# bubustack/bobrapet

Measured on AMD Instinct MI355X. Metric: StoryRuns/sec + p50 step latency, 8-way parallel Story, higher is better.
Workload: dtype bf16; 1 GPU; bench_config=parallel8, global_batch=2165, seq_len=128, parallelism=single, engine=bobraccel-native, branches=8

## Files before the change

### bobrapet_amd/csrc/hip/bindings.cpp

```cpp
#include <torch/extension.h>

#include <c10/hip/HIPStream.h>
#include <hip/hip_runtime.h>

const void* bobra_native_lane_ptr();
bool bobra_native_tensor_get(const std::string& key, at::Tensor* out);
size_t bobra_native_registry_size();
void bobra_native_lane_stats(long*, long*, long*, std::string*);

extern "C" {
void launch_rmsnorm(void*, void*, void*, const void*, int, int, float, bool,
                    hipStream_t);
void launch_silu_mul(void*, const void*, const void*, long, hipStream_t);
void launch_rope(void*, void*, const void*, const void*, int, int, int, int,
                 hipStream_t);
void launch_embed_pool(void*, void*, const void*, const void*, int, int, int,
                       int, hipStream_t);
void launch_add_bf16(void*, const void*, const void*, long, hipStream_t);
void launch_attn_prefill(void*, const void*, const void*, const void*, int,
                         int, int, int, long, float, int, void*, hipStream_t);
void launch_silu_mul_strided(void*, const void*, const void*, long, int, long,
                             hipStream_t);
void launch_rope_qkv(void*, void*, const void*, const void*, const void*, int,
                     int, int, int, long, hipStream_t);
void launch_rope_qkv_decode(void*, void*, void*, const void*, const void*,
                            const void*, int, int, int, int, int, hipStream_t);
void launch_argmax_rows(void*, const void*, int, int, hipStream_t);
void launch_attn_decode(void*, void*, const void*, const void*, const void*,
                        int, int, int, int, int, const void*, float,
                        hipStream_t);
void launch_dbg_mfma(void*, const void*, const void*, hipStream_t);
void launch_attn_prefill_pipe(void*, const void*, const void*, const void*,
                              int, int, int, int, long, float, int, void*,
                              hipStream_t);
void launch_attn_prefill_qrope(void*, const void*, const void*, const void*,
                               int, int, int, int, long, long, const void*,
                               int, float, int, hipStream_t);
void launch_attn_prefill_variant(int, void*, const void*, const void*,
                                 const void*, int, int, int, int, float, int,
                                 hipStream_t);
void launch_gemm_bf16_nt(void*, const void*, const void*, int, int, int,
                         hipStream_t);
void launch_gemv_bf16_nt(void*, const void*, const void*, int, int, int,
                         hipStream_t);
void launch_gemm256(int, void*, const void*, const void*, const void*,
                    const void*, void*, int, int, int, float, float,
                    hipStream_t);
void launch_gemv2(int, void*, const void*, const void*, const void*, int, int,
                  int, float, float, hipStream_t);
void launch_gemm256b_disc(int, void*, const void*, const void*, int, int,
                          int, hipStream_t);
void launch_gemm256w(int, void*, const void*, const void*, const void*,
                     const void*, void*, int, int, int, float, float,
                     hipStream_t);
void launch_gemmsk(int, void*, void*, const void*, const void*, const void*,
                   const void*, void*, int, int, int, float, float,
                   hipStream_t);
long gemmsk_ws_elems(int, int);
void launch_gemm256b(int, void*, const void*, const void*, const void*,
                     const void*, void*, int, int, int, float, float,
                     hipStream_t);
void launch_rowsumsq(void*, const void*, int, int, hipStream_t);
void launch_dbg_attn_core(void*, void*, const void*, const void*, const void*,
                          hipStream_t);
}

namespace {

hipStream_t cur_stream() { return c10::hip::getCurrentHIPStream(); }

void check_bf16(const torch::Tensor& t, const char* name) {
  TORCH_CHECK(t.is_cuda(), name, " must be on the GPU");
  TORCH_CHECK(t.scalar_type() == torch::kBFloat16, name, " must be bf16");
  TORCH_CHECK(t.is_contiguous(), name, " must be contiguous");
}

torch::Tensor rmsnorm(torch::Tensor x, torch::Tensor w, double eps) {
  check_bf16(x, "x");
  check_bf16(w, "w");
  const int H = x.size(-1);
  TORCH_CHECK(H % 8 == 0 && H <= 8192, "rmsnorm: H must be %8==0 and <=8192");
  TORCH_CHECK(w.numel() == H, "rmsnorm: weight shape mismatch");
  auto out = torch::empty_like(x);
  const long rows = x.numel() / H;
  launch_rmsnorm(out.data_ptr(), x.data_ptr(), nullptr, w.data_ptr(),
                 (int)rows, H, (float)eps, false, cur_stream());
  return out;
}

torch::Tensor fused_add_rmsnorm(torch::Tensor x, torch::Tensor residual,
                                torch::Tensor w, double eps) {
  check_bf16(x, "x");
  check_bf16(residual, "residual");
  check_bf16(w, "w");
  const int H = x.size(-1);
  TORCH_CHECK(H % 8 == 0 && H <= 8192, "fused_add_rmsnorm: bad H");
  TORCH_CHECK(residual.sizes() == x.sizes(), "shape mismatch");
  auto out = torch::empty_like(x);
  const long rows = x.numel() / H;
  launch_rmsnorm(out.data_ptr(), x.data_ptr(), residual.data_ptr(),
                 w.data_ptr(), (int)rows, H, (float)eps, true, cur_stream());
  return out;
}

torch::Tensor silu_mul(torch::Tensor gate, torch::Tensor up) {
  check_bf16(gate, "gate");
  check_bf16(up, "up");
  TORCH_CHECK(gate.sizes() == up.sizes(), "silu_mul: shape mismatch");
  TORCH_CHECK(gate.numel() % 8 == 0, "silu_mul: numel must be %8==0");
  auto out = torch::empty_like(gate);
  launch_silu_mul(out.data_ptr(), gate.data_ptr(), up.data_ptr(), gate.numel(),
                  cur_stream());
  return out;
}

void rope_inplace(torch::Tensor q, torch::Tensor k, torch::Tensor cos_t,
                  torch::Tensor sin_t) {
  check_bf16(q, "q");
  check_bf16(k, "k");
  TORCH_CHECK(cos_t.scalar_type() == torch::kFloat32 && cos_t.is_contiguous(),
              "cos must be f32 contiguous");
  TORCH_CHECK(sin_t.scalar_type() == torch::kFloat32 && sin_t.is_contiguous(),
              "sin must be f32 contiguous");
  const int T = q.size(0), Hq = q.size(1), D = q.size(2);
  const int Hk = k.size(1);
  TORCH_CHECK(k.size(0) == T && k.size(2) == D, "rope: q/k shape mismatch");
  TORCH_CHECK(cos_t.size(0) == T && cos_t.size(1) == D / 2, "rope: table shape");
  launch_rope(q.data_ptr(), k.data_ptr(), cos_t.data_ptr(), sin_t.data_ptr(),
              T, Hq, Hk, D, cur_stream());
}

torch::Tensor embed_pool(torch::Tensor table, torch::Tensor ids) {
  check_bf16(table, "table");
  TORCH_CHECK(ids.scalar_type() == torch::kInt32 && ids.is_cuda() &&
                  ids.is_contiguous(),
              "ids must be int32 on GPU");
  const int V = table.size(0), H = table.size(1);
  const int B = ids.size(0), S = ids.size(1);
  TORCH_CHECK(H % 8 == 0 && H <= 8192, "embed_pool: bad H");
  auto out = torch::empty({B, H}, table.options());
  const int nchunk = (S + 7) / 8;
  auto pooled =
      torch::empty({(long)B * nchunk, H}, table.options().dtype(torch::kFloat32));
  if (H % 2048 != 0)
    (void)hipMemsetAsync(pooled.data_ptr(), 0,
                         (size_t)B * nchunk * H * sizeof(float), cur_stream());
  launch_embed_pool(out.data_ptr(), pooled.data_ptr(), table.data_ptr(),
                    ids.data_ptr(), B, S, H, V, cur_stream());
  return out;
}

torch::Tensor add_bf16(torch::Tensor a, torch::Tensor b) {
  check_bf16(a, "a");
  check_bf16(b, "b");
  TORCH_CHECK(a.sizes() == b.sizes() && a.numel() % 8 == 0, "add: bad shapes");
  auto out = torch::empty_like(a);
  launch_add_bf16(out.data_ptr(), a.data_ptr(), b.data_ptr(), a.numel(),
                  cur_stream());
  return out;
}

torch::Tensor attn_prefill(torch::Tensor q, torch::Tensor k, torch::Tensor v,
                           double scale, bool causal) {
  check_bf16(q, "q");
  check_bf16(k, "k");
  const int B = q.size(0), S = q.size(1), Hq = q.size(2), D = q.size(3);
  const int Hkv = k.size(2);
  TORCH_CHECK(D == 128, "attn_prefill: D must be 128");
  TORCH_CHECK(Hq % Hkv == 0, "attn_prefill: Hq must be a multiple of Hkv");
  TORCH_CHECK(k.size(1) == S && v.size(1) == S, "attn_prefill: S mismatch");
  TORCH_CHECK(v.is_cuda() && v.scalar_type() == torch::kBFloat16, "v dtype");
  TORCH_CHECK(v.stride(3) == 1 && v.stride(2) == D, "attn_prefill: v head must be contiguous");
  TORCH_CHECK(v.stride(0) == v.stride(1) * S, "attn_prefill: v batch stride");
  auto out = torch::empty_like(q);
  launch_attn_prefill(out.data_ptr(), q.data_ptr(), k.data_ptr(), v.data_ptr(),
                      B, Hq, Hkv, S, (long)v.stride(1), (float)scale,
                      causal ? 1 : 0, nullptr, cur_stream());
  return out;
}

torch::Tensor attn_prefill_qrope(torch::Tensor q, torch::Tensor k,
                                 torch::Tensor v, torch::Tensor inv_freq,
                                 int64_t pos0, double scale, bool causal) {
  check_bf16(k, "k");
  TORCH_CHECK(q.is_cuda() && q.scalar_type() == torch::kBFloat16, "q dtype");
  const int B = q.size(0), S = q.size(1), Hq = q.size(2), D = q.size(3);
  const int Hkv = k.size(2);
  TORCH_CHECK(D == 128, "attn_prefill_qrope: D must be 128");
  TORCH_CHECK(Hq % Hkv == 0, "attn_prefill_qrope: Hq % Hkv");
  TORCH_CHECK(k.size(1) == S && v.size(1) == S, "attn_prefill_qrope: S mismatch");
  TORCH_CHECK(q.stride(3) == 1 && q.stride(2) == D, "q head must be contiguous");
  TORCH_CHECK(q.stride(0) == q.stride(1) * S, "q batch stride");
  TORCH_CHECK(v.is_cuda() && v.scalar_type() == torch::kBFloat16, "v dtype");
  TORCH_CHECK(v.stride(3) == 1 && v.stride(2) == D, "v head must be contiguous");
  TORCH_CHECK(v.stride(0) == v.stride(1) * S, "v batch stride");
  TORCH_CHECK(inv_freq.is_cuda() && inv_freq.scalar_type() == torch::kFloat32 &&
                  inv_freq.numel() == D / 2 && inv_freq.is_contiguous(),
              "inv_freq must be f32 [D/2] contiguous");
  auto out = torch::empty({B, S, Hq, D}, k.options());
  launch_attn_prefill_qrope(out.data_ptr(), q.data_ptr(), k.data_ptr(),
                            v.data_ptr(), B, Hq, Hkv, S, (long)v.stride(1),
                            (long)q.stride(1), inv_freq.data_ptr(), (int)pos0,
                            (float)scale, causal ? 1 : 0, cur_stream());
  return out;
}

std::vector<torch::Tensor> rope_k_only(torch::Tensor qkv, int64_t Hq,
                                       int64_t Hk, int64_t D,
                                       torch::Tensor cos_t,
                                       torch::Tensor sin_t) {
  check_bf16(qkv, "qkv");
  const long T = qkv.size(0);
  TORCH_CHECK(qkv.is_contiguous(), "rope_k_only: qkv must be contiguous");
  TORCH_CHECK(cos_t.size(0) == T && cos_t.size(1) == D / 2, "rope_k_only tables");
  auto kout = torch::empty({T, Hk, D}, qkv.options());
  const unsigned short* base =
      (const unsigned short*)qkv.data_ptr() + (long)Hq * D;
  launch_rope_qkv(nullptr, kout.data_ptr(), base, cos_t.data_ptr(),
                  sin_t.data_ptr(), (int)T, 0, (int)Hk, (int)D,
                  (long)qkv.size(1), cur_stream());
  return {kout};
}

torch::Tensor attn_prefill_pipe(torch::Tensor q, torch::Tensor k,
                                torch::Tensor v, double scale, bool causal) {
  check_bf16(q, "q");
  check_bf16(k, "k");
  const int B = q.size(0), S = q.size(1), Hq = q.size(2), D = q.size(3);
  const int Hkv = k.size(2);
  TORCH_CHECK(D == 128, "attn_prefill_pipe: D must be 128");
  TORCH_CHECK(Hq % Hkv == 0, "attn_prefill_pipe: Hq % Hkv");
  TORCH_CHECK(k.size(1) == S && v.size(1) == S, "attn_prefill_pipe: S mismatch");
  TORCH_CHECK(v.is_cuda() && v.scalar_type() == torch::kBFloat16, "v dtype");
  TORCH_CHECK(v.stride(3) == 1 && v.stride(2) == D, "v head must be contiguous");
  TORCH_CHECK(v.stride(0) == v.stride(1) * S, "v batch stride");
  auto out = torch::empty_like(q);
  launch_attn_prefill_pipe(out.data_ptr(), q.data_ptr(), k.data_ptr(),
                           v.data_ptr(), B, Hq, Hkv, S, (long)v.stride(1),
                           (float)scale, causal ? 1 : 0, nullptr,
                           cur_stream());
  return out;
}

std::vector<torch::Tensor> attn_prefill_stats(torch::Tensor q, torch::Tensor k,
                                              torch::Tensor v, double scale,
                                              bool causal) {
  check_bf16(q, "q");
  check_bf16(k, "k");
  const int B = q.size(0), S = q.size(1), Hq = q.size(2), D = q.size(3);
  const int Hkv = k.size(2);
  TORCH_CHECK(D == 128, "attn_prefill_stats: D must be 128");
  TORCH_CHECK(Hq % Hkv == 0, "attn_prefill_stats: Hq % Hkv");
  TORCH_CHECK(v.stride(3) == 1 && v.stride(2) == D, "v head must be contiguous");
  auto out = torch::empty_like(q);
  auto stats = torch::empty({B, Hq, S, 2}, q.options().dtype(torch::kFloat32));
  launch_attn_prefill(out.data_ptr(), q.data_ptr(), k.data_ptr(), v.data_ptr(),
                      B, Hq, Hkv, S, (long)v.stride(1), (float)scale,
                      causal ? 1 : 0, stats.data_ptr(), cur_stream());
  return {out, stats};
}

torch::Tensor attn_decode(torch::Tensor q, torch::Tensor kc, torch::Tensor vc,
                          long L, double scale) {
  check_bf16(q, "q");
  check_bf16(kc, "kc");
  check_bf16(vc, "vc");
  const int B = q.size(0), Hq = q.size(1), D = q.size(2);
  const int Hkv = kc.size(1), Smax = kc.size(2);
  TORCH_CHECK(D == 128, "attn_decode: D must be 128");
  TORCH_CHECK(L <= Smax, "attn_decode: L > Smax");
  auto out = torch::empty_like(q);
  void* ws_ptr = nullptr;
  torch::Tensor ws;
  if (!(getenv("BOBRA_DEC_V1") && getenv("BOBRA_DEC_V1")[0] == '1') &&
      Hq / Hkv <= 8) {
    const int nchunk = (Smax + 255) / 256;
    ws = torch::empty({(long)B * Hkv * nchunk * 8 * 130},
                      q.options().dtype(torch::kFloat32));
    ws_ptr = ws.data_ptr();
  }
  launch_attn_decode(out.data_ptr(), ws_ptr, q.data_ptr(), kc.data_ptr(),
                     vc.data_ptr(), B, Hq, Hkv, Smax, (int)L, nullptr,
                     (float)scale, cur_stream());
  return out;
}

torch::Tensor attn_decode_t(torch::Tensor q, torch::Tensor kc,
                            torch::Tensor vc, torch::Tensor L_dev,
                            double scale) {
  check_bf16(q, "q");
  const int B = q.size(0), Hq = q.size(1), D = q.size(2);
  const int Hkv = kc.size(1), Smax = kc.size(2);
  TORCH_CHECK(D == 128, "attn_decode_t: D must be 128");
  TORCH_CHECK(L_dev.scalar_type() == torch::kInt32 && L_dev.is_cuda(),
              "L must be an int32 device scalar");
  auto out = torch::empty_like(q);
  void* ws_ptr = nullptr;
  torch::Tensor ws;
  if (!(getenv("BOBRA_DEC_V1") && getenv("BOBRA_DEC_V1")[0] == '1') &&
      Hq / Hkv <= 8) {
    const int nchunk = (Smax + 255) / 256;
    ws = torch::empty({(long)B * Hkv * nchunk * 8 * 130},
                      q.options().dtype(torch::kFloat32));
    ws_ptr = ws.data_ptr();
  }
  launch_attn_decode(out.data_ptr(), ws_ptr, q.data_ptr(), kc.data_ptr(),
                     vc.data_ptr(), B, Hq, Hkv, Smax, 0, L_dev.data_ptr(),
                     (float)scale, cur_stream());
  return out;
}

torch::Tensor rope_qkv_decode(torch::Tensor qkv, torch::Tensor kc,
                              torch::Tensor vc, torch::Tensor inv_freq,
                              torch::Tensor L_dev, long Hq, long Hkv, long D) {
  check_bf16(qkv, "qkv");
  check_bf16(kc, "kc");
  check_bf16(vc, "vc");
  const int B = qkv.size(0);
  const int Smax = kc.size(2);
  TORCH_CHECK(qkv.size(1) == (Hq + 2 * Hkv) * D, "rope_qkv_decode: row size");
  TORCH_CHECK(inv_freq.scalar_type() == torch::kFloat32 &&
                  inv_freq.is_contiguous() && inv_freq.numel() == D / 2,
              "inv_freq must be f32 [D/2] contiguous");
  TORCH_CHECK(L_dev.scalar_type() == torch::kInt32 && L_dev.is_cuda(),
              "L must be an int32 device scalar");
  auto q_out = torch::empty({(long)B, Hq, D}, qkv.options());
  launch_rope_qkv_decode(q_out.data_ptr(), kc.data_ptr(), vc.data_ptr(),
                         qkv.data_ptr(), inv_freq.data_ptr(), L_dev.data_ptr(),
                         B, (int)Hq, (int)Hkv, (int)D, Smax, cur_stream());
  return q_out;
}

torch::Tensor argmax_rows(torch::Tensor x) {
  check_bf16(x, "x");
  const int N = x.size(-1);
  const int M = x.numel() / N;
  auto ids = torch::empty({(long)M}, x.options().dtype(torch::kLong));
  launch_argmax_rows(ids.data_ptr(), x.data_ptr(), M, N, cur_stream());
  return ids;
}

torch::Tensor silu_mul_strided(torch::Tensor gate_up) {
  check_bf16(gate_up, "gate_up");
  const int two_i = gate_up.size(-1);
  const int inner = two_i / 2;
  TORCH_CHECK(inner % 8 == 0, "silu_mul_strided: I must be %8==0");
  const long rows = gate_up.numel() / two_i;
  auto sizes = gate_up.sizes().vec();
  sizes.back() = inner;
  auto out = torch::empty(sizes, gate_up.options());
  const unsigned short* base = (const unsigned short*)gate_up.data_ptr();
  launch_silu_mul_strided(out.data_ptr(), base, base + inner, rows, inner,
                          (long)two_i, cur_stream());
  return out;
}

std::vector<torch::Tensor> rope_qkv(torch::Tensor qkv, int Hq, int Hk, int D,
                                    torch::Tensor cos_t, torch::Tensor sin_t) {
  check_bf16(qkv, "qkv");
  const long T = qkv.size(0);
  TORCH_CHECK(cos_t.size(0) == T && cos_t.size(1) == D / 2, "rope_qkv tables");
  auto q = torch::empty({T, (long)Hq, (long)D}, qkv.options());
  auto k = torch::empty({T, (long)Hk, (long)D}, qkv.options());
  launch_rope_qkv(q.data_ptr(), k.data_ptr(), qkv.data_ptr(), cos_t.data_ptr(),
                  sin_t.data_ptr(), (int)T, Hq, Hk, D, (long)qkv.size(1),
                  cur_stream());
  return {q, k};
}

torch::Tensor gemm_nt(torch::Tensor a, torch::Tensor b) {
  check_bf16(a, "a");
  check_bf16(b, "b");
  const int M = a.size(0), K = a.size(1), N = b.size(0);
  TORCH_CHECK(b.size(1) == K, "gemm_nt: K mismatch");
  TORCH_CHECK(M % 128 == 0 && N % 128 == 0 && K % 64 == 0,
              "gemm_nt: M,N must be multiples of 128 and K of 64");
  auto c = torch::empty({M, N}, a.options());
  launch_gemm_bf16_nt(c.data_ptr(), a.data_ptr(), b.data_ptr(), M, N, K,
                      cur_stream());
  return c;
}

void check_gemm256(const torch::Tensor& a, const torch::Tensor& b, int M,
                   int N, int K) {
  check_bf16(a, "a");
  check_bf16(b, "b");
  TORCH_CHECK(b.size(1) == K, "gemm256: K mismatch");
  TORCH_CHECK(N % 256 == 0 && K % 32 == 0,
              "gemm256: N must be a multiple of 256 and K of 32");
}

void launch_gemm256_auto(int epi, void* C, const void* A, const void* B,
                         const void* resid, const void* stat_in,
                         void* stat_out, int M, int N, int K, float stat_mul,
                         float stat_eps, hipStream_t st) {
  if (K % 64 == 0)
    launch_gemm256b(epi, C, A, B, resid, stat_in, stat_out, M, N, K, stat_mul,
                    stat_eps, st);
  else
    launch_gemm256(epi, C, A, B, resid, stat_in, stat_out, M, N, K, stat_mul,
                   stat_eps, st);
}

const float* stat_ptr(const c10::optional<torch::Tensor>& stat, int M) {
  if (!stat.has_value()) return nullptr;
  TORCH_CHECK(stat->scalar_type() == torch::kFloat32 && stat->is_contiguous() &&
                  stat->numel() == M,
              "gemm256: row stat must be f32 [M]");
  return (const float*)stat->data_ptr();
}

torch::Tensor gemm256_nt(torch::Tensor a, torch::Tensor b,
                         c10::optional<torch::Tensor> stat, double stat_mul,
                         double stat_eps) {
  const int M = a.size(0), K = a.size(1), N = b.size(0);
  check_gemm256(a, b, M, N, K);
  auto c = torch::empty({M, N}, a.options());
  launch_gemm256_auto(0, c.data_ptr(), a.data_ptr(), b.data_ptr(), nullptr,
                 stat_ptr(stat, M), nullptr, M, N, K, (float)stat_mul,
                 (float)stat_eps, cur_stream());
  return c;
}

torch::Tensor gemm256_nt_disc(torch::Tensor a, torch::Tensor b,
                              int64_t disc) {
  const int M = a.size(0), K = a.size(1), N = b.size(0);
  check_gemm256(a, b, M, N, K);
  TORCH_CHECK(K % 64 == 0, "gemm256_nt_disc: K % 64 required");
  auto c = torch::empty({M, N}, a.options());
  launch_gemm256b_disc((int)disc, c.data_ptr(), a.data_ptr(), b.data_ptr(), M,
                       N, K, cur_stream());
  return c;
}

std::vector<torch::Tensor> gemmsk(torch::Tensor a, torch::Tensor b,
                                  int64_t epi,
                                  c10::optional<torch::Tensor> resid,
                                  c10::optional<torch::Tensor> stat,
                                  double stat_mul, double stat_eps) {
  check_bf16(a, "a");
  check_bf16(b, "b");
  const int M = a.size(0), K = a.size(1), N = b.size(0);
  TORCH_CHECK(M <= 32, "gemmsk: M must be <= 32");
  TORCH_CHECK(N % 64 == 0 && K % 64 == 0, "gemmsk: N%64, K%64 required");
  TORCH_CHECK(a.is_contiguous() && b.is_contiguous(), "gemmsk: contiguous");
  TORCH_CHECK(epi != 2 || (resid && resid->numel() == (long)M * N &&
                           resid->is_contiguous()),
              "gemmsk: resid must be contiguous [M, N]");
  auto c = epi == 1 ? torch::empty({M, N / 2}, a.options())
                    : torch::empty({M, N}, a.options());
  torch::Tensor ws = torch::empty(
// ... 226 lines not shown
```

### bobrapet_amd/csrc/hip/elementwise.hip

```cpp
#include "common.h"


template <bool FUSED_ADD>
__global__ __launch_bounds__(256) void rmsnorm_kernel(
    unsigned short* __restrict__ out,
    unsigned short* __restrict__ x,
    unsigned short* __restrict__ residual,
    const unsigned short* __restrict__ w,
    int H, float eps) {
  const int row = blockIdx.x;
  const long base = (long)row * H;
  const int tid = threadIdx.x;
  const int nthread = blockDim.x;

  float ssq = 0.f;
  float vals[4][8];
  ushort8v raw[4];
  int nchunk = 0;
  for (int c = tid * 8; c < H; c += nthread * 8) {
    ushort8v v = *reinterpret_cast<const ushort8v*>(x + base + c);
    if (FUSED_ADD) {
      ushort8v r = *reinterpret_cast<const ushort8v*>(residual + base + c);
#pragma unroll
      for (int j = 0; j < 8; ++j) {
// ... 2 lines not shown
      }
      *reinterpret_cast<ushort8v*>(residual + base + c) = v;
    } else {
#pragma unroll
      for (int j = 0; j < 8; ++j) vals[nchunk][j] = bf2f(v[j]);
    }
    raw[nchunk] = v;
#pragma unroll
    for (int j = 0; j < 8; ++j) ssq += vals[nchunk][j] * vals[nchunk][j];
    ++nchunk;
  }

  __shared__ float warp_ssq[8];
  ssq = wave_reduce_sum(ssq);
  const int wid = tid / WAVE;
  if ((tid & (WAVE - 1)) == 0) warp_ssq[wid] = ssq;
  __syncthreads();
  float total = 0.f;
#pragma unroll
  for (int i = 0; i < 8; ++i)
    if (i < (nthread + WAVE - 1) / WAVE) total += warp_ssq[i];
  const float scale = rsqrtf(total / (float)H + eps);

  int k = 0;
  for (int c = tid * 8; c < H; c += nthread * 8, ++k) {
    ushort8v wv = *reinterpret_cast<const ushort8v*>(w + c);
    ushort8v o;
#pragma unroll
    for (int j = 0; j < 8; ++j) o[j] = f2bf(vals[k][j] * scale * bf2f(wv[j]));
    *reinterpret_cast<ushort8v*>(out + base + c) = o;
  }
  (void)raw;
}

extern "C" void launch_rmsnorm(void* out, void* x, void* residual, const void* w,
                               int rows, int H, float eps, bool fused_add,
                               hipStream_t stream) {
  dim3 grid(rows), block(256);
  if (fused_add)
    hipLaunchKernelGGL((rmsnorm_kernel<true>), grid, block, 0, stream,
                       (unsigned short*)out, (unsigned short*)x,
                       (unsigned short*)residual, (const unsigned short*)w, H, eps);
  else
    hipLaunchKernelGGL((rmsnorm_kernel<false>), grid, block, 0, stream,
                       (unsigned short*)out, (unsigned short*)x, nullptr,
                       (const unsigned short*)w, H, eps);
}


__global__ __launch_bounds__(256) void silu_mul_kernel(
    unsigned short* __restrict__ out, const unsigned short* __restrict__ gate,
    const unsigned short* __restrict__ up, long n8) {
  for (long i = blockIdx.x * blockDim.x + threadIdx.x; i < n8;
       i += (long)gridDim.x * blockDim.x) {
    ushort8v g = reinterpret_cast<const ushort8v*>(gate)[i];
    ushort8v u = reinterpret_cast<const ushort8v*>(up)[i];
    ushort8v o;
#pragma unroll
    for (int j = 0; j < 8; ++j) {
      float gf = bf2f(g[j]);
      float s = gf / (1.f + __expf(-gf));
      o[j] = f2bf(s * bf2f(u[j]));
    }
    reinterpret_cast<ushort8v*>(out)[i] = o;
  }
}

__global__ __launch_bounds__(256) void silu_mul_strided_kernel(
    unsigned short* __restrict__ out, const unsigned short* __restrict__ gate,
    const unsigned short* __restrict__ up, long rows, int inner,
    long row_stride) {
  const long n8 = rows * (inner / 8);
  const int i8 = inner / 8;
  for (long idx = blockIdx.x * blockDim.x + threadIdx.x; idx < n8;
       idx += (long)gridDim.x * blockDim.x) {
    long r = idx / i8;
    int c = (int)(idx % i8) * 8;
    ushort8v g = *reinterpret_cast<const ushort8v*>(gate + r * row_stride + c);
    ushort8v u = *reinterpret_cast<const ushort8v*>(up + r * row_stride + c);
    ushort8v o;
#pragma unroll
    for (int j = 0; j < 8; ++j) {
      float gf = bf2f(g[j]);
      float sg = gf / (1.f + __expf(-gf));
      o[j] = f2bf(sg * bf2f(u[j]));
    }
    *reinterpret_cast<ushort8v*>(out + r * (long)inner + c) = o;
  }
}

extern "C" void launch_silu_mul_strided(void* out, const void* gate,
                                        const void* up, long rows, int inner,
                                        long row_stride, hipStream_t stream) {
  long n8 = rows * (inner / 8);
  int blocks = (int)((n8 + 255) / 256);
  if (blocks > 2048) blocks = 2048;
  hipLaunchKernelGGL(silu_mul_strided_kernel, dim3(blocks), dim3(256), 0,
                     stream, (unsigned short*)out, (const unsigned short*)gate,
                     (const unsigned short*)up, rows, inner, row_stride);
}

extern "C" void launch_silu_mul(void* out, const void* gate, const void* up,
                                long n, hipStream_t stream) {
  long n8 = n / 8;
  int blocks = (int)((n8 + 255) / 256);
  if (blocks > 2048) blocks = 2048;
  hipLaunchKernelGGL(silu_mul_kernel, dim3(blocks), dim3(256), 0, stream,
                     (unsigned short*)out, (const unsigned short*)gate,
                     (const unsigned short*)up, n8);
}


__global__ __launch_bounds__(256) void rope_kernel(
    unsigned short* __restrict__ q, unsigned short* __restrict__ k,
    const float* __restrict__ cos_t, const float* __restrict__ sin_t, int T,
    int Hq, int Hk, int D) {
  const int half = D / 2;
  const int lane = threadIdx.x & (WAVE - 1);
  const int wave = (blockIdx.x * blockDim.x + threadIdx.x) / WAVE;
  const int total = T * (Hq + Hk);
  const int nwaves = (gridDim.x * blockDim.x) / WAVE;
  for (int idx = wave; idx < total; idx += nwaves) {
    const int t = idx / (Hq + Hk);
    const int h = idx % (Hq + Hk);
    unsigned short* base = (h < Hq) ? q + ((long)t * Hq + h) * D
                                    : k + ((long)t * Hk + (h - Hq)) * D;
    const float* crow = cos_t + (long)t * half;
    const float* srow = sin_t + (long)t * half;
    for (int d = lane; d < half; d += WAVE) {
      float a = bf2f(base[d]);
      float b = bf2f(base[d + half]);
      float c = crow[d], s = srow[d];
      base[d] = f2bf(a * c - b * s);
      base[d + half] = f2bf(b * c + a * s);
    }
  }
}

__global__ __launch_bounds__(256) void rope_qkv_kernel(
    unsigned short* __restrict__ q_out,
    unsigned short* __restrict__ k_out,
    const unsigned short* __restrict__ qkv,
    const float* __restrict__ cos_t, const float* __restrict__ sin_t, int T,
    int Hq, int Hk, int D, long row_stride) {
  const int half = D / 2;
  const int lane = threadIdx.x & (WAVE - 1);
  const int wave = (blockIdx.x * blockDim.x + threadIdx.x) / WAVE;
  const int total = T * (Hq + Hk);
  const int nwaves = (gridDim.x * blockDim.x) / WAVE;
  for (int idx = wave; idx < total; idx += nwaves) {
    const int t = idx / (Hq + Hk);
    const int h = idx % (Hq + Hk);
    const unsigned short* src = qkv + (long)t * row_stride + (long)h * D;
    unsigned short* dst = (h < Hq) ? q_out + ((long)t * Hq + h) * D
                                   : k_out + ((long)t * Hk + (h - Hq)) * D;
    const float* crow = cos_t + (long)t * half;
    const float* srow = sin_t + (long)t * half;
    for (int d = lane; d < half; d += WAVE) {
      float a = bf2f(src[d]);
      float b = bf2f(src[d + half]);
      float c = crow[d], sn = srow[d];
      dst[d] = f2bf(a * c - b * sn);
      dst[d + half] = f2bf(b * c + a * sn);
    }
  }
}

extern "C" void launch_rope_qkv(void* q_out, void* k_out, const void* qkv,
                                const void* cos_t, const void* sin_t, int T,
                                int Hq, int Hk, int D, long row_stride,
                                hipStream_t stream) {
  int total_waves = T * (Hq + Hk);
  int blocks = (total_waves * WAVE + 255) / 256;
  if (blocks > 4096) blocks = 4096;
  hipLaunchKernelGGL(rope_qkv_kernel, dim3(blocks), dim3(256), 0, stream,
                     (unsigned short*)q_out, (unsigned short*)k_out,
                     (const unsigned short*)qkv, (const float*)cos_t,
                     (const float*)sin_t, T, Hq, Hk, D, row_stride);
}

__global__ __launch_bounds__(256) void rope_qkv_decode_kernel(
    unsigned short* __restrict__ q_out,
    unsigned short* __restrict__ kc,
    unsigned short* __restrict__ vc,
    const unsigned short* __restrict__ qkv,
    const float* __restrict__ inv_freq,
    const int* __restrict__ L_dev, int B, int Hq, int Hkv, int D, int Smax) {
  const int L = *L_dev;
  const int half = D / 2;
  const int lane = threadIdx.x & (WAVE - 1);
  const int wave = (blockIdx.x * blockDim.x + threadIdx.x) / WAVE;
  const int nwaves = (gridDim.x * blockDim.x) / WAVE;
  const long row = (long)(Hq + 2 * Hkv) * D;
  const int total = B * (Hq + 2 * Hkv);
  for (int idx = wave; idx < total; idx += nwaves) {
    const int b = idx / (Hq + 2 * Hkv);
    const int h = idx % (Hq + 2 * Hkv);
    const unsigned short* src = qkv + b * row + (long)h * D;
    if (h < Hq + Hkv) {
      unsigned short* dst =
          (h < Hq) ? q_out + ((long)b * Hq + h) * D
                   : kc + (((long)b * Hkv + (h - Hq)) * Smax + L) * D;
      for (int d = lane; d < half; d += WAVE) {
        float a = bf2f(src[d]);
        float bb = bf2f(src[d + half]);
        const float ang = (float)L * inv_freq[d];
        float sn, c;
        __sincosf(ang, &sn, &c);
        dst[d] = f2bf(a * c - bb * sn);
        dst[d + half] = f2bf(bb * c + a * sn);
      }
    } else {
      int hv = h - Hq - Hkv;
      unsigned short* dst = vc + (((long)b * Hkv + hv) * Smax + L) * D;
      for (int d = lane; d < D; d += WAVE) dst[d] = src[d];
    }
  }
}

extern "C" void launch_rope_qkv_decode(void* q_out, void* kc, void* vc,
                                       const void* qkv, const void* inv_freq,
                                       const void* L_dev, int B, int Hq,
                                       int Hkv, int D, int Smax,
                                       hipStream_t stream) {
  int waves_needed = B * (Hq + 2 * Hkv);
  int blocks = (waves_needed + 3) / 4;
  hipLaunchKernelGGL(rope_qkv_decode_kernel, dim3(blocks), dim3(256), 0,
                     stream, (unsigned short*)q_out, (unsigned short*)kc,
                     (unsigned short*)vc, (const unsigned short*)qkv,
                     (const float*)inv_freq, (const int*)L_dev, B, Hq, Hkv, D,
                     Smax);
}

__global__ __launch_bounds__(256) void argmax_rows_kernel(
    long* __restrict__ ids, const unsigned short* __restrict__ x, int N) {
  const int m = blockIdx.x;
  const unsigned short* row = x + (long)m * N;
  const int tid = threadIdx.x;
  float best = -3.4e38f;
  int bi = 0;
  for (int n = tid * 8; n + 7 < N; n += 256 * 8) {
    ushort8v v = *reinterpret_cast<const ushort8v*>(row + n);
#pragma unroll
    for (int j = 0; j < 8; ++j) {
      const float f = bf2f(v[j]);
      if (f > best) {
        best = f;
        bi = n + j;
      }
    }
  }
  for (int n = (N / 8) * 8 + tid; n < N; n += 256) {
    const float f = bf2f(row[n]);
    if (f > best) {
      best = f;
      bi = n;
    }
  }
#pragma unroll
  for (int off = 32; off > 0; off >>= 1) {
    const float ob = __shfl_xor(best, off, WAVE);
    const int oi = __shfl_xor(bi, off, WAVE);
    if (ob > best || (ob == best && oi < bi)) {
      best = ob;
      bi = oi;
    }
  }
  __shared__ float sb[4];
  __shared__ int si[4];
  const int w = tid >> 6;
  if ((tid & (WAVE - 1)) == 0) {
    sb[w] = best;
    si[w] = bi;
  }
  __syncthreads();
  if (tid == 0) {
    for (int i = 1; i < 4; ++i)
      if (sb[i] > best || (sb[i] == best && si[i] < bi)) {
        best = sb[i];
        bi = si[i];
      }
    ids[m] = (long)bi;
  }
}

extern "C" void launch_argmax_rows(void* ids, const void* x, int M, int N,
                                   hipStream_t stream) {
  hipLaunchKernelGGL(argmax_rows_kernel, dim3(M), dim3(256), 0, stream,
                     (long*)ids, (const unsigned short*)x, N);
}

extern "C" void launch_rope(void* q, void* k, const void* cos_t,
                            const void* sin_t, int T, int Hq, int Hk, int D,
                            hipStream_t stream) {
  int total_waves = T * (Hq + Hk);
  int blocks = (total_waves * WAVE + 255) / 256;
  if (blocks > 4096) blocks = 4096;
  hipLaunchKernelGGL(rope_kernel, dim3(blocks), dim3(256), 0, stream,
                     (unsigned short*)q, (unsigned short*)k,
                     (const float*)cos_t, (const float*)sin_t, T, Hq, Hk, D);
}


#define EMB_SCHUNK 8
#define EMB_HSLICE 2048

__global__ __launch_bounds__(256) void embed_pool_sum_kernel(
    float* __restrict__ pooled,
    const unsigned short* __restrict__ table,
    const int* __restrict__ ids,
    int B, int S, int H, int V) {
  const int nslice = (H + EMB_HSLICE - 1) / EMB_HSLICE;
  const int nchunk = (S + EMB_SCHUNK - 1) / EMB_SCHUNK;
  int wg = blockIdx.x;
  const int b = wg / (nchunk * nslice);
  const int chunk = (wg / nslice) % nchunk;
  const int slice = wg % nslice;
  const int tid = threadIdx.x;
  const int h0 = slice * EMB_HSLICE + tid * 8;
  if (h0 + 8 > H) return;

  float acc[8] = {};
  const int s0 = chunk * EMB_SCHUNK;
  const int s_end = min(s0 + EMB_SCHUNK, S);
  int id_reg[EMB_SCHUNK];
#pragma unroll
  for (int i = 0; i < EMB_SCHUNK; ++i) {
    int sidx = s0 + i;
    id_reg[i] = (sidx < s_end) ? ids[(long)b * S + sidx] : -1;
  }
  ushort8v rows[EMB_SCHUNK];
#pragma unroll
  for (int i = 0; i < EMB_SCHUNK; ++i) {
    int id = id_reg[i];
    rows[i] = (id >= 0 && id < V)
                  ? *reinterpret_cast<const ushort8v*>(table + (long)id * H + h0)
                  : ushort8v{0, 0, 0, 0, 0, 0, 0, 0};
  }
#pragma unroll
  for (int i = 0; i < EMB_SCHUNK; ++i)
#pragma unroll
    for (int j = 0; j < 8; ++j) acc[j] += bf2f(rows[i][j]);
  float* dst = pooled + (((long)b * nchunk + chunk) * H) + h0;
  float4v lo, hi;
#pragma unroll
  for (int j = 0; j < 4; ++j) { lo[j] = acc[j]; hi[j] = acc[j + 4]; }
  *reinterpret_cast<float4v*>(dst) = lo;
  *reinterpret_cast<float4v*>(dst + 4) = hi;
}

__global__ __launch_bounds__(256) void embed_pool_norm_kernel(
    unsigned short* __restrict__ out, const float* __restrict__ pooled, int S,
    int H, int nchunk) {
  const int b = blockIdx.x;
  const int tid = threadIdx.x;
  const float inv_s = 1.f / (float)S;
  float vals[4][8];
  float ssq = 0.f;
  int k = 0;
  for (int c = tid * 8; c < H; c += 256 * 8, ++k) {
    float sum[8] = {};
    for (int ch = 0; ch < nchunk; ++ch) {
      const float* src = pooled + (((long)b * nchunk + ch) * H) + c;
      const float4v lo = *reinterpret_cast<const float4v*>(src);
      const float4v hic = *reinterpret_cast<const float4v*>(src + 4);
#pragma unroll
      for (int j = 0; j < 4; ++j) { sum[j] += lo[j]; sum[j + 4] += hic[j]; }
    }
#pragma unroll
    for (int j = 0; j < 8; ++j) vals[k][j] = sum[j] * inv_s;
#pragma unroll
    for (int j = 0; j < 8; ++j) ssq += vals[k][j] * vals[k][j];
  }
  __shared__ float warp_ssq[8];
  ssq = wave_reduce_sum(ssq);
  if ((tid & (WAVE - 1)) == 0) warp_ssq[tid / WAVE] = ssq;
  __syncthreads();
  float total = 1e-12f;
#pragma unroll
  for (int i = 0; i < 4; ++i) total += warp_ssq[i];
  const float inv_norm = rsqrtf(total);
  k = 0;
  for (int c = tid * 8; c < H; c += 256 * 8, ++k) {
    ushort8v o;
#pragma unroll
    for (int j = 0; j < 8; ++j) o[j] = f2bf(vals[k][j] * inv_norm);
    *reinterpret_cast<ushort8v*>(out + (long)b * H + c) = o;
  }
}

extern "C" void launch_embed_pool(void* out, void* pooled_f32, const void* table,
                                  const void* ids, int B, int S, int H, int V,
                                  hipStream_t stream) {
  const int nslice = (H + EMB_HSLICE - 1) / EMB_HSLICE;
  const int nchunk = (S + EMB_SCHUNK - 1) / EMB_SCHUNK;
  hipLaunchKernelGGL(embed_pool_sum_kernel, dim3(B * nchunk * nslice), dim3(256),
                     0, stream, (float*)pooled_f32,
                     (const unsigned short*)table, (const int*)ids, B, S, H, V);
  hipLaunchKernelGGL(embed_pool_norm_kernel, dim3(B), dim3(256), 0, stream,
                     (unsigned short*)out, (const float*)pooled_f32, S, H,
                     nchunk);
}


__global__ __launch_bounds__(256) void add_kernel(
    unsigned short* __restrict__ out, const unsigned short* __restrict__ a,
    const unsigned short* __restrict__ b, long n8) {
  for (long i = blockIdx.x * blockDim.x + threadIdx.x; i < n8;
       i += (long)gridDim.x * blockDim.x) {
    ushort8v x = reinterpret_cast<const ushort8v*>(a)[i];
    ushort8v y = reinterpret_cast<const ushort8v*>(b)[i];
    ushort8v o;
#pragma unroll
    for (int j = 0; j < 8; ++j) o[j] = f2bf(bf2f(x[j]) + bf2f(y[j]));
    reinterpret_cast<ushort8v*>(out)[i] = o;
  }
}

extern "C" void launch_add_bf16(void* out, const void* a, const void* b, long n,
                                hipStream_t stream) {
  long n8 = n / 8;
  int blocks = (int)((n8 + 255) / 256);
  if (blocks > 2048) blocks = 2048;
  hipLaunchKernelGGL(add_kernel, dim3(blocks), dim3(256), 0, stream,
                     (unsigned short*)out, (const unsigned short*)a,
                     (const unsigned short*)b, n8);
}
```

### bobrapet_amd/csrc/hip/native_engrams.cpp

```cpp
#include <ATen/ATen.h>
#include <c10/hip/HIPCachingAllocator.h>
#include <c10/hip/HIPStream.h>
#include <hip/hip_runtime.h>

#include <deque>
#include <mutex>
#include <string>
#include <unordered_map>
#include <vector>
#include <chrono>

#include "../core/jvalue.h"
#include "../core/native_lane.h"

extern "C" void launch_embed_pool(void*, void*, const void*, const void*, int,
                                  int, int, int, hipStream_t);

namespace {

using bobraccel::JArray;
using bobraccel::JObject;
using bobraccel::JValue;
using bobraccel::NativeLane;

double now_s() {
  return std::chrono::duration<double>(
             std::chrono::steady_clock::now().time_since_epoch())
      .count();
}

int64_t jint(const JValue& v, const char* key, int64_t dflt) {
  if (!v.is_object()) return dflt;
  const JObject& o = v.as_object();
  auto it = o.find(key);
  if (it == o.end()) return dflt;
  if (it->second.is_int()) return it->second.as_int();
  if (it->second.is_double()) return (int64_t)it->second.as_double();
  return dflt;
}

struct Entry {
  at::Tensor t;
  hipEvent_t ready = nullptr;
};

struct Ticket {
  hipEvent_t ev = nullptr;
  JValue out;
  double t0 = 0;
};

struct LaneState {
  std::mutex mu;
  std::unordered_map<std::string, Entry> registry;
  std::deque<std::string> order;
  std::unordered_map<long, Ticket> tickets;
  long next_key = 1;
  long next_ticket = 1;
  std::unordered_map<std::string, at::Tensor> cache;
  std::vector<std::vector<c10::hip::HIPStream>> streams;
  int rr = 0;
  long launches = 0;
  long fallbacks = 0;
  long failures = 0;
  std::string last_error;
};

LaneState& S() {
  static LaneState s;
  return s;
}

constexpr size_t kRegistryCap = 16384;

c10::hip::HIPStream pick_stream(int device) {
  LaneState& s = S();
  if ((int)s.streams.size() <= device) s.streams.resize(device + 1);
  auto& pool = s.streams[device];
  if (pool.empty()) {
    for (int i = 0; i < 4; ++i)
      pool.push_back(c10::hip::getStreamFromPool(false, device));
  }
  return pool[(s.rr++) & 3];
}

std::string register_tensor(at::Tensor t, hipEvent_t ev) {
  LaneState& s = S();
  std::string key = "native/t-" + std::to_string(s.next_key++);
  if (s.order.size() >= kRegistryCap) {
    const std::string& old = s.order.front();
    auto it = s.registry.find(old);
    if (it != s.registry.end()) {
      if (it->second.ready) hipEventDestroy(it->second.ready);
      s.registry.erase(it);
    }
    s.order.pop_front();
  }
  s.registry[key] = Entry{std::move(t), ev};
  s.order.push_back(key);
  return key;
}

JValue tensor_ref(const std::string& key, const at::Tensor& t) {
  JObject meta;
  meta["key"] = key;
  meta["kind"] = std::string("tensor");
  meta["dtype"] = std::string(t.scalar_type() == at::kBFloat16 ? "bfloat16"
                              : t.scalar_type() == at::kFloat  ? "float32"
                                                               : "other");
  JArray shape;
  for (auto d : t.sizes()) shape.push_back((int64_t)d);
  meta["shape"] = std::move(shape);
  meta["device"] = std::string("cuda:") + std::to_string(t.get_device());
  meta["size"] = (int64_t)(t.numel() * t.element_size());
  JObject ref;
  ref["$storageRef"] = std::move(meta);
  return JValue(std::move(ref));
}

at::Tensor cached_table(int64_t vocab, int64_t dim, int64_t seed, int device) {
  LaneState& s = S();
  std::string key = "tab/" + std::to_string(vocab) + "/" + std::to_string(dim) +
                    "/" + std::to_string(seed) + "/" + std::to_string(device);
  auto it = s.cache.find(key);
  if (it != s.cache.end()) return it->second;
  auto gen = at::detail::createCPUGenerator((uint64_t)seed);
  at::Tensor cpu = at::empty({vocab, dim}, at::dtype(at::kFloat));
  cpu.normal_(0.0, 0.05, gen);
  at::Tensor t = cpu.to(at::device(at::kCUDA).dtype(at::kBFloat16),
                        false);
  if (t.get_device() != device)
    t = t.to(at::Device(at::kCUDA, device));
  s.cache[key] = t;
  return t;
}

at::Tensor cached_ids(int64_t vocab, int64_t batch, int64_t seq, int64_t sd,
                      int device) {
  LaneState& s = S();
  std::string key = "ids/" + std::to_string(vocab) + "/" + std::to_string(batch) +
                    "/" + std::to_string(seq) + "/" + std::to_string(sd) + "/" +
                    std::to_string(device);
  auto it = s.cache.find(key);
  if (it != s.cache.end()) return it->second;
  auto gen = at::detail::createCPUGenerator((uint64_t)sd);
  at::Tensor cpu = at::randint(0, vocab, {batch, seq}, gen,
                               at::dtype(at::kLong));
  at::Tensor t = cpu.to(at::device(at::Device(at::kCUDA, device)).dtype(at::kInt));
  s.cache[key] = t;
  return t;
}


long embed_launch(const JValue& cfg, const JValue& inp, int device) {
  LaneState& s = S();
  std::lock_guard<std::mutex> g(s.mu);
  const int64_t dim = jint(inp, "dim", jint(cfg, "dim", 4096));
  const int64_t vocab = jint(inp, "vocab", jint(cfg, "vocab", 32000));
  const int64_t seed = jint(cfg, "seed", 7);
  if (inp.is_object() && inp.as_object().count("ids"))
    return 0;
  const int64_t batch = jint(inp, "batch", jint(cfg, "batch", 32));
  const int64_t seq = jint(inp, "seqLen", jint(cfg, "seqLen", 128));
  const int64_t sd = jint(inp, "seed", 0);
  if (dim % 8 != 0 || dim > 8192) return 0;

  at::Tensor table = cached_table(vocab, dim, seed, device);
  at::Tensor ids = cached_ids(vocab, batch, seq, sd, device);

  auto stream = pick_stream(device);
  c10::hip::setCurrentHIPStream(stream);
  at::Tensor out = at::empty({batch, dim},
                             at::device(at::Device(at::kCUDA, device))
                                 .dtype(at::kBFloat16));
  const int nchunk = (int)((seq + 7) / 8);
  at::Tensor pooled = at::zeros({batch * nchunk, dim},
                                at::device(at::Device(at::kCUDA, device))
                                    .dtype(at::kFloat));
  launch_embed_pool(out.data_ptr(), pooled.data_ptr(), table.data_ptr(),
                    ids.data_ptr(), (int)batch, (int)seq, (int)dim, (int)vocab,
                    stream.stream());
  hipEvent_t ev;
  hipEventCreateWithFlags(&ev, hipEventDisableTiming);
  hipEventRecord(ev, stream.stream());

  std::string key = register_tensor(out, ev);
  JObject o;
  o["batch"] = (int64_t)batch;
  o["dim"] = (int64_t)dim;
  o["embeddings"] = tensor_ref(key, out);
  long tk = s.next_ticket++;
  s.tickets[tk] = Ticket{ev, JValue(std::move(o)), now_s()};
  return tk;
}

long join_launch(const JValue& cfg, const JValue& inp, int device) {
  (void)cfg;
  LaneState& s = S();
  std::lock_guard<std::mutex> g(s.mu);
  if (!inp.is_object()) return 0;
  const JObject& o = inp.as_object();
  std::vector<std::string> keys;
  auto collect_ref = [&](const JValue& ref) -> bool {
    if (!ref.is_object()) return false;
    auto it = ref.as_object().find("$storageRef");
    if (it == ref.as_object().end() || !it->second.is_object()) return false;
    auto kit = it->second.as_object().find("key");
    if (kit == it->second.as_object().end() || !kit->second.is_string())
      return false;
    const std::string& k = kit->second.as_string();
    if (k.rfind("native/", 0) != 0) return false;
    keys.push_back(k);
    return true;
  };
  auto bit = o.find("branches");
  if (bit != o.end() && bit->second.is_object()) {
    for (const auto& [name, bout] : bit->second.as_object()) {
      if (!bout.is_object()) continue;
      auto e = bout.as_object().find("embeddings");
      if (e == bout.as_object().end())
        e = bout.as_object().find("logits");
      if (e == bout.as_object().end()) continue;
      if (!collect_ref(e->second)) return 0;
    }
  } else {
    auto rit = o.find("refs");
    if (rit == o.end() || !rit->second.is_array()) return 0;
    for (const auto& r : rit->second.as_array())
      if (!collect_ref(r)) return 0;
  }
  if (keys.empty()) return 0;

  std::vector<at::Tensor> parts;
  std::vector<hipEvent_t> waits;
  for (const std::string& k : keys) {
    auto it = s.registry.find(k);
    if (it == s.registry.end()) {
      s.failures++;
      s.last_error = "native join: ref " + k + " not in the lane registry";
      return -1;
    }
    parts.push_back(it->second.t.reshape({-1, it->second.t.size(-1)}));
    if (it->second.ready) waits.push_back(it->second.ready);
  }
  const int dev = parts[0].get_device();
  auto stream = pick_stream(dev);
  for (hipEvent_t ev : waits) hipStreamWaitEvent(stream.stream(), ev, 0);
  c10::hip::setCurrentHIPStream(stream);
  at::Tensor local = at::cat(parts, 0);
  for (auto& p : parts)
    c10::hip::HIPCachingAllocator::recordStream(p.storage().data_ptr(), stream);
  hipEvent_t ev;
  hipEventCreateWithFlags(&ev, hipEventDisableTiming);
  hipEventRecord(ev, stream.stream());
  std::string key = register_tensor(local, ev);

  JObject out;
  out["rows"] = (int64_t)local.size(0);
  out["dim"] = (int64_t)local.size(-1);
  out["worldRows"] = (int64_t)local.size(0);
  out["world"] = (int64_t)1;
  out["joined"] = tensor_ref(key, local);
  long tk = s.next_ticket++;
  s.tickets[tk] = Ticket{ev, JValue(std::move(out)), now_s()};
  return tk;
}

long fail_ticket(const std::string& msg) {
  LaneState& s = S();
  std::lock_guard<std::mutex> g(s.mu);
  s.failures++;
  s.last_error = msg;
  long tk = s.next_ticket++;
  Ticket t;
  t.ev = nullptr;
  t.out = JValue(msg);
  s.tickets[tk] = std::move(t);
  return tk;
}

long lane_launch(void*, int kind, const JValue* cfg, const JValue* input,
                 int device) {
  long r = 0;
  try {
    if (kind == 1)
      r = embed_launch(*cfg, *input, device);
    else if (kind == 2)
      r = join_launch(*cfg, *input, device);
  } catch (const std::exception& e) {
    return fail_ticket(std::string("native lane: ") + e.what());
  }
  LaneState& s = S();
  std::string err;
  {
    std::lock_guard<std::mutex> g(s.mu);
    if (r > 0) s.launches++;
    if (r == 0) s.fallbacks++;
    if (r >= 0) return r;
    err = s.last_error;
  }
  return fail_ticket(err);
}

int lane_poll(void*, long ticket, JValue* out, std::string* err) {
  LaneState& s = S();
  std::lock_guard<std::mutex> g(s.mu);
  auto it = s.tickets.find(ticket);
  if (it == s.tickets.end()) {
    *err = "unknown native ticket";
    return -1;
  }
  if (it->second.ev == nullptr) {
    *err = it->second.out.is_string() ? it->second.out.as_string()
                                      : "native lane failure";
    s.tickets.erase(it);
    return -1;
  }
  hipError_t rc = hipEventQuery(it->second.ev);
  if (rc == hipErrorNotReady) return 0;
  if (rc != hipSuccess) {
    *err = std::string("hip error: ") + hipGetErrorString(rc);
    s.tickets.erase(it);
    return -1;
  }
  JValue o = std::move(it->second.out);
  if (o.is_object())
    o.as_object()["latencyMs"] = (now_s() - it->second.t0) * 1000.0;
  *out = std::move(o);
  s.tickets.erase(it);
  return 1;
}

void lane_free_key(void*, const char* key) {
  LaneState& s = S();
  std::lock_guard<std::mutex> g(s.mu);
  auto it = s.registry.find(key);
  if (it == s.registry.end()) return;
  if (it->second.ready) hipEventDestroy(it->second.ready);
  s.registry.erase(it);
}

NativeLane g_lane{1, nullptr, &lane_launch, &lane_poll, &lane_free_key};

}


const void* bobra_native_lane_ptr() { return &g_lane; }

bool bobra_native_tensor_get(const std::string& key, at::Tensor* out) {
  LaneState& s = S();
  at::Tensor t;
  hipEvent_t ev = nullptr;
  {
    std::lock_guard<std::mutex> g(s.mu);
    auto it = s.registry.find(key);
    if (it == s.registry.end()) return false;
    t = it->second.t;
    ev = it->second.ready;
  }
  if (ev) (void)hipEventSynchronize(ev);
  *out = t;
  return true;
}

size_t bobra_native_registry_size() {
  LaneState& s = S();
  std::lock_guard<std::mutex> g(s.mu);
  return s.registry.size();
}

void bobra_native_lane_stats(long* launches, long* fallbacks, long* failures,
                             std::string* last_error) {
  LaneState& s = S();
  std::lock_guard<std::mutex> g(s.mu);
  *launches = s.launches;
  *fallbacks = s.fallbacks;
  *failures = s.failures;
  *last_error = s.last_error;
}
```

Measured before the change: 3528 runs/s.

## Fuse embedding gather-sum and L2 norm into one per-row kernel

Replaces the two-kernel embed pool (a chunked gather-sum writing fp32 partials to global memory, then a normalize pass) with one 1024-thread kernel per batch row. Token ids are staged in shared memory, gathers run with 16 loads in flight, and partials are reduced in shared memory before the L2 normalisation. This removes the fp32 scratch allocation, its zero-fill memset, a second launch and the global round trip. In exchange there is only one block per batch row with large shared memory use, so occupancy may drop, and rows with H above 8192 or lanes that do not divide the thread count would be handled differently.

```diff
diff --git a/bobrapet_amd/csrc/hip/bindings.cpp b/bobrapet_amd/csrc/hip/bindings.cpp
--- a/bobrapet_amd/csrc/hip/bindings.cpp
+++ b/bobrapet_amd/csrc/hip/bindings.cpp
@@ -14,8 +14,8 @@
 void launch_silu_mul(void*, const void*, const void*, long, hipStream_t);
 void launch_rope(void*, void*, const void*, const void*, int, int, int, int,
                  hipStream_t);
-void launch_embed_pool(void*, void*, const void*, const void*, int, int, int,
-                       int, hipStream_t);
+void launch_embed_pool(void*, const void*, const void*, int, int, int, int,
+                       hipStream_t);
 void launch_add_bf16(void*, const void*, const void*, long, hipStream_t);
 void launch_attn_prefill(void*, const void*, const void*, const void*, int,
                          int, int, int, long, float, int, void*, hipStream_t);
@@ -139,14 +139,8 @@
   const int B = ids.size(0), S = ids.size(1);
   TORCH_CHECK(H % 8 == 0 && H <= 8192, "embed_pool: bad H");
   auto out = torch::empty({B, H}, table.options());
-  const int nchunk = (S + 7) / 8;
-  auto pooled =
-      torch::empty({(long)B * nchunk, H}, table.options().dtype(torch::kFloat32));
-  if (H % 2048 != 0)
-    (void)hipMemsetAsync(pooled.data_ptr(), 0,
-                         (size_t)B * nchunk * H * sizeof(float), cur_stream());
-  launch_embed_pool(out.data_ptr(), pooled.data_ptr(), table.data_ptr(),
-                    ids.data_ptr(), B, S, H, V, cur_stream());
+  launch_embed_pool(out.data_ptr(), table.data_ptr(), ids.data_ptr(), B, S, H,
+                    V, cur_stream());
   return out;
 }
 
diff --git a/bobrapet_amd/csrc/hip/elementwise.hip b/bobrapet_amd/csrc/hip/elementwise.hip
--- a/bobrapet_amd/csrc/hip/elementwise.hip
+++ b/bobrapet_amd/csrc/hip/elementwise.hip
@@ -328,104 +328,102 @@
 }
 
 
-#define EMB_SCHUNK 8
-#define EMB_HSLICE 2048
-
-__global__ __launch_bounds__(256) void embed_pool_sum_kernel(
-    float* __restrict__ pooled,
+#define EMB_THREADS 1024
+#define EMB_IDS_TILE 1024
+#define EMB_INFLIGHT 16
+
+__global__ __launch_bounds__(EMB_THREADS) void embed_pool_row_kernel(
+    unsigned short* __restrict__ out,
     const unsigned short* __restrict__ table,
     const int* __restrict__ ids,
-    int B, int S, int H, int V) {
-  const int nslice = (H + EMB_HSLICE - 1) / EMB_HSLICE;
-  const int nchunk = (S + EMB_SCHUNK - 1) / EMB_SCHUNK;
-  int wg = blockIdx.x;
-  const int b = wg / (nchunk * nslice);
-  const int chunk = (wg / nslice) % nchunk;
-  const int slice = wg % nslice;
-  const int tid = threadIdx.x;
-  const int h0 = slice * EMB_HSLICE + tid * 8;
-  if (h0 + 8 > H) return;
-
-  float acc[8] = {};
-  const int s0 = chunk * EMB_SCHUNK;
-  const int s_end = min(s0 + EMB_SCHUNK, S);
-  int id_reg[EMB_SCHUNK];
-#pragma unroll
-  for (int i = 0; i < EMB_SCHUNK; ++i) {
-    int sidx = s0 + i;
-    id_reg[i] = (sidx < s_end) ? ids[(long)b * S + sidx] : -1;
-  }
-  ushort8v rows[EMB_SCHUNK];
-#pragma unroll
-  for (int i = 0; i < EMB_SCHUNK; ++i) {
-    int id = id_reg[i];
-    rows[i] = (id >= 0 && id < V)
-                  ? *reinterpret_cast<const ushort8v*>(table + (long)id * H + h0)
-                  : ushort8v{0, 0, 0, 0, 0, 0, 0, 0};
-  }
-#pragma unroll
-  for (int i = 0; i < EMB_SCHUNK; ++i)
-#pragma unroll
-    for (int j = 0; j < 8; ++j) acc[j] += bf2f(rows[i][j]);
-  float* dst = pooled + (((long)b * nchunk + chunk) * H) + h0;
-  float4v lo, hi;
-#pragma unroll
-  for (int j = 0; j < 4; ++j) { lo[j] = acc[j]; hi[j] = acc[j + 4]; }
-  *reinterpret_cast<float4v*>(dst) = lo;
-  *reinterpret_cast<float4v*>(dst + 4) = hi;
-}
-
-__global__ __launch_bounds__(256) void embed_pool_norm_kernel(
-    unsigned short* __restrict__ out, const float* __restrict__ pooled, int S,
-    int H, int nchunk) {
+    int S, int H, int V) {
+  __shared__ float part[EMB_THREADS * 8];
+  __shared__ int sid[EMB_IDS_TILE];
+  __shared__ float wave_ssq[EMB_THREADS / WAVE];
+
   const int b = blockIdx.x;
   const int tid = threadIdx.x;
+  const int lanes = H >> 3;
+  const int G = max(EMB_THREADS / lanes, 1);
+  const int g = tid / lanes;
+  const int h0 = (tid - g * lanes) * 8;
+  const bool gathers = g < G && V > 0;
+
+  float acc[8] = {};
+  for (int s0 = 0; s0 < S; s0 += EMB_IDS_TILE) {
+    const int n = min(EMB_IDS_TILE, S - s0);
+    if (s0 > 0) __syncthreads();
+    if (tid < n) sid[tid] = ids[(long)b * S + s0 + tid];
+    __syncthreads();
+    if (gathers) {
+      for (int p = g; p < n; p += G * EMB_INFLIGHT) {
+        ushort8v rows[EMB_INFLIGHT];
+        bool ok[EMB_INFLIGHT];
+#pragma unroll
+        for (int i = 0; i < EMB_INFLIGHT; ++i) {
+          const int q = p + i * G;
+          const int id = sid[min(q, n - 1)];
+          ok[i] = q < n && id >= 0 && id < V;
+          rows[i] = *reinterpret_cast<const ushort8v*>(
+              table + (long)(ok[i] ? id : 0) * H + h0);
+        }
+#pragma unroll
+        for (int i = 0; i < EMB_INFLIGHT; ++i)
+#pragma unroll
+          for (int j = 0; j < 8; ++j)
+            acc[j] += ok[i] ? bf2f(rows[i][j]) : 0.f;
+      }
+    }
+  }
+
+  float4v lo, hi;
+#pragma unroll
+  for (int j = 0; j < 4; ++j) { lo[j] = acc[j]; hi[j] = acc[j + 4]; }
+  *reinterpret_cast<float4v*>(part + tid * 8) = lo;
+  *reinterpret_cast<float4v*>(part + tid * 8 + 4) = hi;
+  __syncthreads();
+
+  const bool owner = tid < lanes;
   const float inv_s = 1.f / (float)S;
-  float vals[4][8];
+  float vals[8];
   float ssq = 0.f;
-  int k = 0;
-  for (int c = tid * 8; c < H; c += 256 * 8, ++k) {
+  if (owner) {
     float sum[8] = {};
-    for (int ch = 0; ch < nchunk; ++ch) {
-      const float* src = pooled + (((long)b * nchunk + ch) * H) + c;
-      const float4v lo = *reinterpret_cast<const float4v*>(src);
-      const float4v hic = *reinterpret_cast<const float4v*>(src + 4);
-#pragma unroll
-      for (int j = 0; j < 4; ++j) { sum[j] += lo[j]; sum[j + 4] += hic[j]; }
-    }
-#pragma unroll
-    for (int j = 0; j < 8; ++j) vals[k][j] = sum[j] * inv_s;
-#pragma unroll
-    for (int j = 0; j < 8; ++j) ssq += vals[k][j] * vals[k][j];
-  }
-  __shared__ float warp_ssq[8];
+    for (int gg = 0; gg < G; ++gg) {
+      const float* src = part + (gg * lanes + tid) * 8;
+      const float4v a = *reinterpret_cast<const float4v*>(src);
+      const float4v c = *reinterpret_cast<const float4v*>(src + 4);
+#pragma unroll
+      for (int j = 0; j < 4; ++j) { sum[j] += a[j]; sum[j + 4] += c[j]; }
+    }
+#pragma unroll
+    for (int j = 0; j < 8; ++j) {
+      vals[j] = sum[j] * inv_s;
+      ssq += vals[j] * vals[j];
+    }
+  }
   ssq = wave_reduce_sum(ssq);
-  if ((tid & (WAVE - 1)) == 0) warp_ssq[tid / WAVE] = ssq;
+  if ((tid & (WAVE - 1)) == 0) wave_ssq[tid / WAVE] = ssq;
   __syncthreads();
   float total = 1e-12f;
 #pragma unroll
-  for (int i = 0; i < 4; ++i) total += warp_ssq[i];
+  for (int i = 0; i < EMB_THREADS / WAVE; ++i) total += wave_ssq[i];
   const float inv_norm = rsqrtf(total);
-  k = 0;
-  for (int c = tid * 8; c < H; c += 256 * 8, ++k) {
+  if (owner) {
     ushort8v o;
 #pragma unroll
-    for (int j = 0; j < 8; ++j) o[j] = f2bf(vals[k][j] * inv_norm);
-    *reinterpret_cast<ushort8v*>(out + (long)b * H + c) = o;
-  }
-}
-
-extern "C" void launch_embed_pool(void* out, void* pooled_f32, const void* table,
-                                  const void* ids, int B, int S, int H, int V,
+    for (int j = 0; j < 8; ++j) o[j] = f2bf(vals[j] * inv_norm);
+    *reinterpret_cast<ushort8v*>(out + (long)b * H + h0) = o;
+  }
+}
+
+extern "C" void launch_embed_pool(void* out, const void* table, const void* ids,
+                                  int B, int S, int H, int V,
                                   hipStream_t stream) {
-  const int nslice = (H + EMB_HSLICE - 1) / EMB_HSLICE;
-  const int nchunk = (S + EMB_SCHUNK - 1) / EMB_SCHUNK;
-  hipLaunchKernelGGL(embed_pool_sum_kernel, dim3(B * nchunk * nslice), dim3(256),
-                     0, stream, (float*)pooled_f32,
-                     (const unsigned short*)table, (const int*)ids, B, S, H, V);
-  hipLaunchKernelGGL(embed_pool_norm_kernel, dim3(B), dim3(256), 0, stream,
-                     (unsigned short*)out, (const float*)pooled_f32, S, H,
-                     nchunk);
+  if (B == 0 || H == 0) return;
+  hipLaunchKernelGGL(embed_pool_row_kernel, dim3(B), dim3(EMB_THREADS), 0,
+                     stream, (unsigned short*)out, (const unsigned short*)table,
+                     (const int*)ids, S, H, V);
 }
 
 
diff --git a/bobrapet_amd/csrc/hip/native_engrams.cpp b/bobrapet_amd/csrc/hip/native_engrams.cpp
--- a/bobrapet_amd/csrc/hip/native_engrams.cpp
+++ b/bobrapet_amd/csrc/hip/native_engrams.cpp
@@ -13,8 +13,8 @@
 #include "../core/jvalue.h"
 #include "../core/native_lane.h"
 
-extern "C" void launch_embed_pool(void*, void*, const void*, const void*, int,
-                                  int, int, int, hipStream_t);
+extern "C" void launch_embed_pool(void*, const void*, const void*, int, int,
+                                  int, int, hipStream_t);
 
 namespace {
 
@@ -173,12 +173,8 @@
   at::Tensor out = at::empty({batch, dim},
                              at::device(at::Device(at::kCUDA, device))
                                  .dtype(at::kBFloat16));
-  const int nchunk = (int)((seq + 7) / 8);
-  at::Tensor pooled = at::zeros({batch * nchunk, dim},
-                                at::device(at::Device(at::kCUDA, device))
-                                    .dtype(at::kFloat));
-  launch_embed_pool(out.data_ptr(), pooled.data_ptr(), table.data_ptr(),
-                    ids.data_ptr(), (int)batch, (int)seq, (int)dim, (int)vocab,
+  launch_embed_pool(out.data_ptr(), table.data_ptr(), ids.data_ptr(),
+                    (int)batch, (int)seq, (int)dim, (int)vocab,
                     stream.stream());
   hipEvent_t ev;
   hipEventCreateWithFlags(&ev, hipEventDisableTiming);
```

Measured after the change: 4604 runs/s (median of 6 runs). +30.5%, better.
